# fogleman/sdf

Hardware: AMD Instinct MI355X
Metric: grid voxels/sec (sampled + meshed), canonical CSG example (higher is better)
Workload: dtype f64; 1 GPU; example @ samples=2**27 -> 512x512x512 grid, sparse=True, batch_size=32; batches=4096, skipped=2352, empty=120, nonempty=1624, triangles=2945152, parallelism=single GPU

## Files before the change

sdf_amd/csrc/sdf_device.h:

```cpp
#pragma once
#include <hip/hip_runtime.h>
#include <stdint.h>
#include <type_traits>

#include "sdf_interp.h"
#include "sdf_mc33.h"
#include "sdf_interval.h"
#include "sdf_slab.h"

namespace sdfk {

struct McTables {
    unsigned char ntri[256];
    unsigned char amb[256];
    signed char tri[256][16];
    signed char mc33[MC33_FLAT_SIZE];
};

struct MeshCounters {
    unsigned long long n_pruned;
    unsigned long long n_eval;
    unsigned int work_counter;
    unsigned int overflow;
    unsigned int n_empty, n_nonempty;
    unsigned long long n_ambiguous;
    unsigned long long n_sampled;
    unsigned long long total;
    unsigned long long cell_cursor;
    unsigned long long list_cursor;
    unsigned long long t_first_inv, t_last, clk_cycles, clk_ticks;
    unsigned long long n_raw;
    int nwork, work_begin, work_end, pad_;
};
enum { MESH_COUNTERS_RESET_BYTES = 112 };

struct GridDesc {
    const double *X, *Y, *Z;
    int nx, ny, nz;
    int bs;
    int nbx, nby, nbz;
};

struct MeshArgs {
    GridDesc g;
    const McTables *mc;
    const int *worklist;
    unsigned char *kinds;
    unsigned long long *status;
    double *out;
    unsigned long long out_cap;
    MeshCounters *ctr;
    int bits_off;
    int list_off;
    int list_cap;
    unsigned long long *prof;
    int tape_stride;
    int n_instr;
    float *park;
    int park_cap;
    unsigned park_spins;
    const unsigned char *cull;
    int slot_bytes;
    int stage_off;
    int compact;
    double *xf;
    int xf_cap;
    float *raw;
    long long raw_cap;
    int twopass;
    struct ItemDesc *desc;
    unsigned *cells;
    unsigned *tlist;
    unsigned long long cells_cap, tlist_cap;
    const int *block_item;
    const int *order;
    int tail;
};
enum { MESH_TAIL_MAX = 255 };

struct ItemDesc {
    unsigned ntri, ncells;
    unsigned long long list_off, cell_off;
    double xf[6];
};

enum { MESH_PARK_DEPTH = 16 };
enum { MESH_LDS_SUMS2 = 128, MESH_LDS_NTRI = 192, MESH_LDS_AXES = MESH_LDS_NTRI + 256, MESH_LDS_PEND = MESH_LDS_AXES + 800, MESH_LDS_TRI = MESH_LDS_PEND + 64 * MESH_PARK_DEPTH,
       MESH_LDS_VOL = MESH_LDS_TRI + 256 * 5 * 2 };

__device__ __forceinline__ void batch_origin(const GridDesc &g, int b, int &ox, int &oy, int &oz, int &lx, int &ly, int &lz) {
    const int ibz = b % g.nbz, iby = (b / g.nbz) % g.nby, ibx = b / (g.nbz * g.nby);
    ox = ibx * g.bs; oy = iby * g.bs; oz = ibz * g.bs;
    lx = min(g.bs + 1, g.nx - ox); ly = min(g.bs + 1, g.ny - oy); lz = min(g.bs + 1, g.nz - oz);
}

__device__ __forceinline__ int fast_div(int i, float inv_d) { return (int)(((float)i + 0.5f) * inv_d); }

template <int BLOCK>
__device__ __forceinline__ int block_exclusive_scan(int v, int *wave_sums, int &total) {
    const int lane = threadIdx.x & 63, wid = threadIdx.x >> 6;
    int inc = v;
    inc += __builtin_amdgcn_update_dpp(0, inc, 0x111, 0xf, 0xf, false);
    inc += __builtin_amdgcn_update_dpp(0, inc, 0x112, 0xf, 0xf, false);
    inc += __builtin_amdgcn_update_dpp(0, inc, 0x114, 0xf, 0xf, false);
    inc += __builtin_amdgcn_update_dpp(0, inc, 0x118, 0xf, 0xf, false);
    inc += __builtin_amdgcn_update_dpp(0, inc, 0x142, 0xa, 0xf, false);
    inc += __builtin_amdgcn_update_dpp(0, inc, 0x143, 0xc, 0xf, false);
    if (lane == 63) wave_sums[wid] = inc;
    __syncthreads();
    int base = 0, tot = 0;
#pragma unroll
    for (int w = 0; w < BLOCK / 64; w++) { const int s = wave_sums[w]; if (w < wid) base += s; tot += s; }
    total = tot;
    __syncthreads();
    return base + inc - v;
}

template <int BLOCK>
__device__ __forceinline__ int block_exclusive_scan1(int v, int *wave_sums, int &total) {
    int t = threadIdx.x;
    asm volatile("" : "+v"(t));
    const int lane = t & 63, wid = __builtin_amdgcn_readfirstlane(t >> 6);
    int inc = v;
    inc += __builtin_amdgcn_update_dpp(0, inc, 0x111, 0xf, 0xf, false);
    inc += __builtin_amdgcn_update_dpp(0, inc, 0x112, 0xf, 0xf, false);
    inc += __builtin_amdgcn_update_dpp(0, inc, 0x114, 0xf, 0xf, false);
    inc += __builtin_amdgcn_update_dpp(0, inc, 0x118, 0xf, 0xf, false);
    inc += __builtin_amdgcn_update_dpp(0, inc, 0x142, 0xa, 0xf, false);
    inc += __builtin_amdgcn_update_dpp(0, inc, 0x143, 0xc, 0xf, false);
    if (lane == 63) wave_sums[wid] = inc;
    __syncthreads();
    static_assert(BLOCK / 64 <= 16, "a row of 16 lanes holds the wave totals");
    const int l16 = lane & 15;
    int tot = l16 < BLOCK / 64 ? wave_sums[l16] : 0, base = l16 < wid ? tot : 0;
    tot += __builtin_amdgcn_update_dpp(0, tot, 0x111, 0xf, 0xf, false);   base += __builtin_amdgcn_update_dpp(0, base, 0x111, 0xf, 0xf, false);
    tot += __builtin_amdgcn_update_dpp(0, tot, 0x112, 0xf, 0xf, false);   base += __builtin_amdgcn_update_dpp(0, base, 0x112, 0xf, 0xf, false);
    tot += __builtin_amdgcn_update_dpp(0, tot, 0x114, 0xf, 0xf, false);   base += __builtin_amdgcn_update_dpp(0, base, 0x114, 0xf, 0xf, false);
    tot += __builtin_amdgcn_update_dpp(0, tot, 0x118, 0xf, 0xf, false);   base += __builtin_amdgcn_update_dpp(0, base, 0x118, 0xf, 0xf, false);
    total = __builtin_amdgcn_readlane(tot, 15);
    return __builtin_amdgcn_readlane(base, 15) + inc - v;
}

template <int BLOCK>
__device__ __forceinline__ int block_exclusive_count(bool p, int *wave_sums, int &total) {
    const unsigned long long m = __ballot(p);
    const int below = (int)__builtin_amdgcn_mbcnt_hi((unsigned)(m >> 32), __builtin_amdgcn_mbcnt_lo((unsigned)m, 0u));
    const int wid = threadIdx.x >> 6;
    if ((threadIdx.x & 63) == 0) wave_sums[wid] = __popcll(m);
    __syncthreads();
    int base = 0, tot = 0;
#pragma unroll
    for (int w = 0; w < BLOCK / 64; w++) { const int s = wave_sums[w]; if (w < wid) base += s; tot += s; }
    total = tot;
    __syncthreads();
    return base + below;
}

__device__ __forceinline__ unsigned plane_bits(const float *v, int s0, int s1) {
    return (v[0] > 0.0f ? 1u : 0u) | (v[s1] > 0.0f ? 2u : 0u) | (v[s0] > 0.0f ? 4u : 0u) | (v[s0 + s1] > 0.0f ? 8u : 0u);
}
__device__ __forceinline__ unsigned spread4(unsigned s) { return (s & 1u) | ((s & 2u) << 1) | ((s & 4u) << 2) | ((s & 8u) << 3); }

__device__ __forceinline__ unsigned cell_config(const unsigned long long *rb, int i2) {
    unsigned cfg = 0;
#pragma unroll
    for (int q = 0; q < 4; q++) cfg |= ((unsigned)(rb[q] >> i2) & 3u) << (2 * q);
    return cfg;
}

#ifndef SDF_TAPE_WARM
#define SDF_TAPE_WARM 1
#endif
#ifndef SDF_FAST_VERTEX
#define SDF_FAST_VERTEX 1
#endif
__device__ __forceinline__ float mc_edge_pos(double vlo, double vhi, double ibase) {
    const double eps = 2.220446049250313e-16;
    const double a = eps + fabs(vlo), b = eps + fabs(vhi);
    float pf;
#if SDF_FAST_VERTEX
    const double sab = a + b;
    double r = __builtin_amdgcn_rcp(sab);
    r = fma(fma(-sab, r, 1.0), r, r);
    r = fma(fma(-sab, r, 1.0), r, r);
    double tq = a * r;
    tq = fma(fma(-sab, tq, a), r, tq);
    const double q = ibase + tq;
    const float f_lo = (float)(q - 0x1p-44), f_hi = (float)(q + 0x1p-44);
    pf = f_lo;
    if (__builtin_expect(!(f_lo == f_hi), 0))
#endif
    {
        const double wlo = 1.0 / a, whi = 1.0 / b;
        const double t = whi / (wlo + whi);
        pf = (float)(ibase + t);
    }
    return pf;
}
__device__ __forceinline__ void mc_vertex(const float *v, int s0, int s1, int i0, int i1, int i2, int e, float *o) {
    const int axis = e >> 2, oa = (e >> 1) & 1, ob = e & 1;
    int o0, o1, o2, stride;
    if (axis == 0) { o0 = 0; o1 = oa; o2 = ob; stride = s0; }
    else if (axis == 1) { o0 = oa; o1 = 0; o2 = ob; stride = s1; }
    else { o0 = oa; o1 = ob; o2 = 0; stride = 1; }
    const int base = o0 * s0 + o1 * s1 + o2;
    const float pf = mc_edge_pos((double)v[base], (double)v[base + stride], (double)(axis == 0 ? i0 : (axis == 1 ? i1 : i2)));
    o[0] = axis == 0 ? pf : (float)(i0 + o0); o[1] = axis == 1 ? pf : (float)(i1 + o1); o[2] = axis == 2 ? pf : (float)(i2 + o2);
}

struct TileView {
    const float *smp;
    const unsigned *colinfo;
    int lyz, lz;
    bool sparse;
    __device__ __forceinline__ float at(int ix, int iy, int iz) const {
        if (!sparse) return smp[ix * lyz + iy * lz + iz];
        const unsigned c = colinfo[(ix >> 1) * 17 + (iy >> 1)];
        const int k = (int)(c >> 17) + __popc(c & ((1u << (iz >> 1)) - 1u));
        return smp[8 * k + ((ix & 1) << 2) + ((iy & 1) << 1) + (iz & 1)];
    }
    __device__ __forceinline__ void cell(int i0, int i1, int i2, float *c8) const {
#pragma unroll
        for (int q = 0; q < 8; q++) c8[q] = at(i0 + (q >> 2), i1 + ((q >> 1) & 1), i2 + (q & 1));
    }
};
__device__ __forceinline__ void mc_vertex_view(const TileView &vw, int i0, int i1, int i2, int e, float *o) {
    const int axis = e >> 2, oa = (e >> 1) & 1, ob = e & 1;
    const int o0 = axis == 0 ? 0 : oa, o1 = axis == 0 ? oa : (axis == 1 ? 0 : ob), o2 = axis == 2 ? 0 : ob;
    const int x = i0 + o0, y = i1 + o1, z = i2 + o2;
    const float vlo = vw.at(x, y, z), vhi = vw.at(x + (axis == 0 ? 1 : 0), y + (axis == 1 ? 1 : 0), z + (axis == 2 ? 1 : 0));
    const float pf = mc_edge_pos((double)vlo, (double)vhi, (double)(axis == 0 ? i0 : (axis == 1 ? i1 : i2)));
    o[0] = axis == 0 ? pf : (float)x; o[1] = axis == 1 ? pf : (float)y; o[2] = axis == 2 ? pf : (float)z;
}

struct Tri16Sink {
    double *out;
    float *raw;
    long long raw_cap;
// ... 56 lines not shown
    bool use_first = true;
    for (unsigned spins = 0; spins < max_spins;) {
        constexpr int NW = 4;
        unsigned long long sw[NW];
        const int nwin = use_first ? 1 : NW;
        if (use_first) sw[0] = first;
        else {
#pragma unroll
            for (int k = 0; k < NW; k++) {
                const int j = idx - 64 * k - lane;
                sw[k] = j >= w_begin ? __hip_atomic_load(&status[j], __ATOMIC_RELAXED, __HIP_MEMORY_SCOPE_AGENT)
                                     : MESH_FLAG_PFX;
            }
        }
        use_first = false;
        bool wait = false;
#pragma unroll
        for (int k = 0; k < NW; k++) {
            if (k >= nwin || wait) break;
            const unsigned flag = (unsigned)(sw[k] >> 62);
            const unsigned long long pending = __ballot(flag == 0), is_pfx = __ballot(flag == 2);
            if (is_pfx) {
                const int p = __ffsll((long long)is_pfx) - 1;
                if (pending & ((1ull << p) - 1ull)) { wait = true; break; }
                acc += lane <= p ? (sw[k] & MESH_VAL_MASK) : 0ull;
                const unsigned long long excl = wave_sum_u64(acc);
                if (lane == 0) __hip_atomic_store(&status[w], MESH_FLAG_PFX | (excl + total), __ATOMIC_RELAXED, __HIP_MEMORY_SCOPE_AGENT);
                return excl;
            }
            if (pending) { wait = true; break; }
            acc += sw[k] & MESH_VAL_MASK;
            idx -= 64;
        }
        if (wait) { __builtin_amdgcn_s_sleep(1); spins++; }
    }
    return max_spins < (1u << 24) ? MESH_NOT_READY : ~0ull;
}
#define MESH_SPIN_FOREVER (1u << 24)

__device__ __noinline__ void mc33_triangle(const float *corner, int s0, int s1, int i0, int i1, int i2,
                                           const signed char *tab, int j, float *o) {
    double lv[8];
    int off;
    mc33_load_cell(corner, s0, s1, lv);
    const int n = mc33_cell(lv, tab, &off);
    if (j >= n) { for (int q = 0; q < 9; q++) o[q] = 0.0f; return; }
    const signed char lew_edge[12] = {8, 5, 9, 4, 10, 7, 11, 6, 0, 1, 3, 2};
    for (int q = 0; q < 3; q++) {
        const int e = tab[off + 3 * j + 2 - q];
        if (e == 12) mc33_centre_vertex(lv, i0, i1, i2, o + 3 * q);
        else mc_vertex(corner, s0, s1, i0, i1, i2, lew_edge[e], o + 3 * q);
    }
}

struct TileTasks {
    int lx, ly, lz, lyz, nvox;
    float inv_lyz, inv_lz;
    bool regular;
    int ntask;
    __device__ __forceinline__ TileTasks(int lx_, int ly_, int lz_) : lx(lx_), ly(ly_), lz(lz_) {
        lyz = ly * lz; nvox = lx * lyz;
        inv_lyz = 1.0f / (float)lyz; inv_lz = 1.0f / (float)lz;
        regular = lx == 33 && ly == 33 && lz == 33;
        ntask = regular ? 563 : (nvox + 63) >> 6;
    }
    __device__ __forceinline__ bool sample(int task, int lane, int &ix, int &iy, int &iz) const {
        if (!regular) {
            const int i = min(task * 64 + lane, nvox - 1);
            ix = fast_div(i, inv_lyz); const int r = i - ix * lyz; iy = fast_div(r, inv_lz); iz = r - iy * lz;
            return task * 64 + lane < nvox;
        }
        if (task < 512) { ix = 4 * (task >> 6) + (lane >> 4); iy = 4 * ((task >> 3) & 7) + ((lane >> 2) & 3); iz = 4 * (task & 7) + (lane & 3); return true; }
        if (task < 530) { const int p = min((task - 512) * 64 + lane, 1088); ix = 32; iy = fast_div(p, 1.0f / 33.0f); iz = p - 33 * iy; return (task - 512) * 64 + lane < 1089; }
        if (task < 547) { const int p = min((task - 530) * 64 + lane, 1055); iy = 32; ix = fast_div(p, 1.0f / 33.0f); iz = p - 33 * ix; return (task - 530) * 64 + lane < 1056; }
        const int p = (task - 547) * 64 + lane; iz = 32; ix = p >> 5; iy = p & 31; return true;
    }
};

enum { CULL_UNIT_CAP = 3072, CULL_ULIST = 8, CULL_SBYTES = CULL_ULIST, CULL_SSTATE = CULL_ULIST + 2 * CULL_UNIT_CAP, CULL_COLINFO = CULL_SSTATE + 1024,
       CULL_RECORD = CULL_COLINFO + 1160,
       CULL_MSTATE = CULL_RECORD, CULL_GSTATE = CULL_MSTATE + 64, CULL_ELIST = CULL_GSTATE + 512, CULL_PACC = CULL_ELIST + 1024,
       CULL_SCRATCH = CULL_PACC + 64 };
static_assert(CULL_RECORD % 8 == 0 && CULL_SSTATE % 8 == 0 && CULL_COLINFO % 8 == 0, "the record is copied in words; its state rows are read as u64");
__device__ __forceinline__ bool cull_sample(const unsigned short *units, int task, int lane, int lx, int ly, int lz, int &ix, int &iy, int &iz) {
    const unsigned u = units[8 * task + (lane >> 3)];
    const int x = (int)((u >> 9) & 62u) + ((lane >> 2) & 1), y = (int)((u >> 4) & 62u) + ((lane >> 1) & 1), z = (int)((u << 1) & 62u) + (lane & 1);
    const bool ok = x < lx && y < ly && z < lz;
    ix = ok ? x : 0; iy = ok ? y : 0; iz = ok ? z : 0;
    return ok;
}
template <int BLOCK, bool FULL, bool RARE>
__device__ __forceinline__ int cull_tasks(const uint32_t *wcode, const double *consts, int n_instr_w, int lx, int ly, int lz,
                                       const double *axes, double *ia_state, int ia_bytes, unsigned char *scratch, int *wave_sums,
                                       int ia_np, int ia_nd, unsigned long long *prof = nullptr, int levels = 3) {
    const int tid = threadIdx.x;
    long long tprev = prof ? clock64() : 0;
    unsigned *pacc = reinterpret_cast<unsigned *>(scratch + CULL_PACC);
    if (prof && tid == 0) for (int k = 0; k < 12; k++) pacc[k] = 0;
#define SDF_CULL_PROF(K) do { if (prof && tid == 0) { const long long tn = clock64(); pacc[(K) - 16] += (unsigned)(tn - tprev); tprev = tn; } } while (0)
    const int c0 = lx - 1, c1 = ly - 1, c2 = lz - 1;
    const int per_pass = min(BLOCK, ia_bytes / ((6 * ia_np + 2 * ia_nd) * 8)) & ~63;
    if (c0 <= 0 || c1 <= 0 || c2 <= 0 || per_pass < 64) return -1;
    unsigned short *ulist = reinterpret_cast<unsigned short *>(scratch + CULL_ULIST);
    unsigned char *sstate = scratch + CULL_SBYTES;
    static_assert(2 * CULL_UNIT_CAP >= 4096, "the byte states lie over the unit list");
    unsigned char *mstate = scratch + CULL_MSTATE;
    unsigned char *gstate = scratch + CULL_GSTATE;
    unsigned short *elist = reinterpret_cast<unsigned short *>(scratch + CULL_ELIST);
    auto box_state = [&](int x0, int x1, int y0, int y1, int z0, int z1) -> unsigned char {
        Ival bx{axes[x0], axes[min(x1, c0)]}, by{axes[33 + y0], axes[33 + min(y1, c1)]}, bz{axes[66 + z0], axes[66 + min(z1, c2)]};
        if (bx.lo > bx.hi) { const double t = bx.lo; bx.lo = bx.hi; bx.hi = t; }
        if (by.lo > by.hi) { const double t = by.lo; by.lo = by.hi; by.hi = t; }
        if (bz.lo > bz.hi) { const double t = bz.lo; bz.lo = bz.hi; bz.hi = t; }
        if (ia::bad(bx) || ia::bad(by) || ia::bad(bz)) { bx = by = bz = ia::top(); }
        const Ival v = ia_run_tape<false, FULL, RARE>(wcode, consts, nullptr, nullptr, n_instr_w, bx, by, bz, true,
                                          IaShared{ia_state, ia_np, per_pass}, ia_nd, nullptr);
        return v.lo > 1e-30 ? 1 : (v.hi < -1e-30 ? 2 : 0);
    };
    int phase = 0, e0 = 0, nev = 0;
    for (;;) {
        if (phase == 1 && e0 >= nev) {
            __syncthreads();
            SDF_CULL_PROF(19);
            int nund = 0;
            for (int g0 = 0; levels >= 3 && g0 < 512; g0 += BLOCK) {
                const int gi = g0 + tid;
                const bool und = gi < 512 && gstate[gi] == 0;
                int n;
                const int pos = nund + block_exclusive_count<BLOCK>(und, wave_sums, n);
                if (und) elist[pos] = (unsigned short)gi;
                nund += n;
            }
            for (int h = tid; h < 4096; h += BLOCK) {
                const int h0 = h >> 8, h1 = (h >> 4) & 15, h2 = h & 15;
                const bool exists = 2 * h0 < c0 && 2 * h1 < c1 && 2 * h2 < c2;
                sstate[h] = exists ? gstate[((h0 >> 1) * 8 + (h1 >> 1)) * 8 + (h2 >> 1)] : 1;
            }
            __syncthreads();
            phase = 2; e0 = 0; nev = 8 * nund;
        }
        if (phase == 2 && e0 >= nev) break;
        const bool run = phase == 0 ? tid < 64 : (tid < per_pass && e0 + (tid & ~63) < nev);
        int target = 0, x0, y0, z0, ext;
        bool live;
        if (phase == 0) {
            const int m0 = tid >> 4, m1 = (tid >> 2) & 3, m2 = tid & 3;
            live = 8 * m0 < c0 && 8 * m1 < c1 && 8 * m2 < c2;
            x0 = live ? 8 * m0 : 0; y0 = live ? 8 * m1 : 0; z0 = live ? 8 * m2 : 0; ext = 8;
        } else if (phase == 1) {
            live = e0 + tid < nev;
            target = run ? (int)elist[min(e0 + tid, nev - 1)] : 0;
            x0 = 4 * (target >> 6); y0 = 4 * ((target >> 3) & 7); z0 = 4 * (target & 7); ext = 4;
        } else {
            const int e = min(e0 + tid, nev - 1);
            const int gq = run ? (int)elist[e >> 3] : 0, ch = e & 7;
            const int h0 = 2 * (gq >> 6) + (ch >> 2), h1 = 2 * ((gq >> 3) & 7) + ((ch >> 1) & 1), h2 = 2 * (gq & 7) + (ch & 1);
            live = e0 + tid < nev && 2 * h0 < c0 && 2 * h1 < c1 && 2 * h2 < c2;
            target = (h0 * 16 + h1) * 16 + h2;
            x0 = live ? 2 * h0 : 0; y0 = live ? 2 * h1 : 0; z0 = live ? 2 * h2 : 0; ext = 2;
        }
        if (run) {
            const unsigned char st = box_state(x0, x0 + ext, y0, y0 + ext, z0, z0 + ext);
            if (phase == 0) mstate[tid & 63] = live ? st : 1;
            else if (live) (phase == 1 ? gstate : sstate)[target] = st;
        }
        if (phase != 0) { if (prof && tid == 0) pacc[7]++; e0 += per_pass; continue; }
        SDF_CULL_PROF(17);
        __syncthreads();
        for (int g0 = 0; g0 < 512; g0 += BLOCK) {
            const int gi = g0 + tid;
            const int a0 = gi >> 6, a1 = (gi >> 3) & 7, a2 = gi & 7;
            const bool exists = gi < 512 && 4 * a0 < c0 && 4 * a1 < c1 && 4 * a2 < c2;
            const unsigned char ms = exists ? mstate[((a0 >> 1) * 4 + (a1 >> 1)) * 4 + (a2 >> 1)] : 1;
            if (gi < 512) gstate[gi] = ms;
            int n;
            const int pos = nev + block_exclusive_count<BLOCK>(ms == 0, wave_sums, n);
            if (ms == 0) elist[pos] = (unsigned short)gi;
            nev += n;
        }
        __syncthreads();
        SDF_CULL_PROF(18);
        if (prof && tid == 0) pacc[6] = (unsigned)nev;
        phase = 1; e0 = 0;
    }
    __syncthreads();
    SDF_CULL_PROF(20);
    unsigned short *ub = reinterpret_cast<unsigned short *>(scratch + CULL_GSTATE);
    for (int r = tid; r < 256; r += BLOCK) {
        const unsigned long long lo8 = *reinterpret_cast<const unsigned long long *>(sstate + 16 * r);
        const unsigned long long hi8 = *reinterpret_cast<const unsigned long long *>(sstate + 16 * r + 8);
        unsigned m = 0, pk = 0;
        SDF_UNROLL for (int k = 0; k < 8; k++) { m |= ((lo8 >> (8 * k)) & 255ull) == 0ull ? 1u << k : 0u; pk |= (unsigned)((lo8 >> (8 * k)) & 3ull) << (2 * k); }
        SDF_UNROLL for (int k = 0; k < 8; k++) { m |= ((hi8 >> (8 * k)) & 255ull) == 0ull ? 256u << k : 0u; pk |= (unsigned)((hi8 >> (8 * k)) & 3ull) << (2 * k + 16); }
        ub[r] = (unsigned short)m;
        reinterpret_cast<unsigned *>(scratch + CULL_SSTATE)[r] = pk;
    }
    __syncthreads();
    const int nu0 = (lx + 1) >> 1, nu1 = (ly + 1) >> 1, nu2 = (lz + 1) >> 1;
    int nlisted = 0;
    unsigned *colinfo = reinterpret_cast<unsigned *>(scratch + CULL_COLINFO);
    for (int q0 = 0; q0 < 17 * 17; q0 += BLOCK) {
        const int q = q0 + tid, u0 = q / 17, u1 = q - 17 * u0;
        unsigned um = 0;
        if (q < 17 * 17 && u0 < nu0 && u1 < nu1) {
            unsigned m = 0;
            for (int d0 = 0; d0 < 2; d0++)
                for (int d1 = 0; d1 < 2; d1++) {
                    const int h0 = u0 - d0, h1 = u1 - d1;
                    if (h0 >= 0 && h0 < 16 && h1 >= 0 && h1 < 16) m |= ub[h0 * 16 + h1];
                }
            um = (m | (m << 1)) & ((1u << nu2) - 1u);
        }
        int n;
        int pos = nlisted + block_exclusive_scan<BLOCK>(__popc(um), wave_sums, n);
        nlisted += n;
        if (q < 17 * 17) colinfo[q] = um | ((unsigned)min(pos, 32767) << 17);
        if (nlisted <= CULL_UNIT_CAP) {
            while (um) {
                const int u2 = __ffs((int)um) - 1;
                um &= um - 1u;
                ulist[pos++] = (unsigned short)((u0 << 10) | (u1 << 5) | u2);
            }
        }
    }
    SDF_CULL_PROF(24);
    if (nlisted > CULL_UNIT_CAP) { __syncthreads(); return -1; }
    if (tid < 8 && nlisted + tid < ((nlisted + 7) & ~7)) ulist[nlisted + tid] = 0xFFFFu;
    if (tid == 0) reinterpret_cast<unsigned short *>(scratch)[0] = (unsigned short)nlisted;
    __syncthreads();
    SDF_CULL_PROF(25);
#undef SDF_CULL_PROF
    return (nlisted + 7) >> 3;
}

#ifndef SDF_SOUP_NT
#define SDF_SOUP_NT 0
#endif
#if SDF_SOUP_NT
#define SDF_SOUP_STORE(PTR, VAL) __builtin_nontemporal_store((VAL), (PTR))
#else
#define SDF_SOUP_STORE(PTR, VAL) (*(PTR) = (VAL))
#endif

enum { MESH_SLOT_HDR = 1232, MESH_SLOT_COLINFO = 64, MESH_STAGE_BYTES = 32 * 9 * 4 };

template <typename T, bool FULL, int NP, int ND, int NS, int BLOCK, bool TWOPASS, bool PROF>
__device__ __forceinline__ void mesh_rounds(const uint32_t *__restrict__ code, const T *__restrict__ consts) {
    typedef __attribute__((address_space(4))) const MeshArgs KArgs;
    static_assert(sizeof(const uint32_t *) + sizeof(const T *) == 16 && alignof(MeshArgs) <= 16, "MeshArgs sits at byte 16 of the kernel arguments");
    KArgs *ap = (KArgs *)((__attribute__((address_space(4))) const char *)__builtin_amdgcn_kernarg_segment_ptr() + 16);
#define KA (*ap)
#define SDF_SINK (Tri16Sink{KA.out, KA.raw, KA.raw_cap, &KA.ctr->n_raw})
    typedef Vec<T, NS> V;
    constexpr int RPT = 1024 / BLOCK;
    constexpr int MESH_CELL_CHUNKS = 2;
    extern __shared__ __attribute__((aligned(16))) unsigned char smem[];
    int *wave_sums = reinterpret_cast<int *>(smem);
    int *bcast = wave_sums + 16;
    unsigned char *ntri_lds = smem + MESH_LDS_NTRI;
    double *axes = reinterpret_cast<double *>(smem + MESH_LDS_AXES);
    float *vol = reinterpret_cast<float *>(smem + MESH_LDS_VOL);
    unsigned long long *bits = reinterpret_cast<unsigned long long *>(smem + KA.bits_off);
    unsigned *wlist = reinterpret_cast<unsigned *>(smem + KA.list_off);
    int tid = threadIdx.x;
#define SDF_FRESH() do { asm volatile("" : "+v"(tid), "+s"(ap)); \
                         bits = reinterpret_cast<unsigned long long *>(smem + KA.bits_off); wlist = reinterpret_cast<unsigned *>(smem + KA.list_off); } while (0)
#define SDF_PROF_ON (PROF && KA.prof)
    auto grid = [&]() { GridDesc g_; g_.X = KA.g.X; g_.Y = KA.g.Y; g_.Z = KA.g.Z; g_.nx = KA.g.nx; g_.ny = KA.g.ny; g_.nz = KA.g.nz; g_.bs = KA.g.bs;
                        g_.nbx = KA.g.nbx; g_.nby = KA.g.nby; g_.nbz = KA.g.nbz; return g_; };
    unsigned short *tri_lds = reinterpret_cast<unsigned short *>(smem + MESH_LDS_TRI);

    if (tid < 256) ntri_lds[tid] = (unsigned char)(KA.mc->ntri[tid] | (KA.mc->amb[tid] << 7));
    if (!TWOPASS)
        for (int i = tid; i < 256 * 5; i += BLOCK) {
            const int cfg = i / 5, j = i - 5 * cfg;
            const signed char *t3 = &KA.mc->tri[cfg][3 * j];
            tri_lds[i] = (unsigned short)(((unsigned)t3[0] & 15u) | (((unsigned)t3[1] & 15u) << 4) | (((unsigned)t3[2] & 15u) << 8));
        }

    for (int i = tid; i < (int)((KA.list_off - KA.bits_off) >> 3); i += BLOCK) bits[i] = 0ull;
    const int work_begin = KA.ctr->work_begin, work_end = KA.ctr->work_end;
    if (SDF_PROF_ON && tid == 0) KA.prof[64 + 4 * blockIdx.x] = wall_clock64();
    if (tid == 0) {
        const unsigned long long tw = wall_clock64();
        atomicMax(&KA.ctr->t_first_inv, ~tw);
        if (blockIdx.x == 0) { KA.ctr->clk_cycles = (unsigned long long)clock64(); KA.ctr->clk_ticks = tw; }
    }
    long long tprev = SDF_PROF_ON ? clock64() : 0;
#define SDF_PROF(K) do { if (SDF_PROF_ON && tid == 0) { const long long tn = clock64(); atomicAdd(&KA.prof[K], (unsigned long long)(tn - tprev)); tprev = tn; } } while (0)
    auto settle = [&](int w_, unsigned long long excl, unsigned long long total_) {
        if (excl == ~0ull) atomicOr(&KA.ctr->overflow, 2u);
        else if (excl + total_ > KA.out_cap) atomicOr(&KA.ctr->overflow, 1u);
        if (w_ == work_end - 1 && excl != ~0ull) KA.ctr->total = excl + total_;
    };
    auto my_park = [&]() -> float * { return KA.park ? KA.park + (size_t)blockIdx.x * (size_t)MESH_PARK_DEPTH * (size_t)KA.park_cap * 9 : nullptr; };
    int pq_head = 0, pq_count = 0;
    unsigned char *pend_base = smem + MESH_LDS_PEND;
    auto pend_xf = [&](int k) { return reinterpret_cast<double *>(pend_base + 64 * k); };
    auto pend_wt = [&](int k) { return reinterpret_cast<int *>(pend_base + 64 * k + 48); };
    auto place_parked = [&](unsigned long long pre_pend, bool must, int need) {
        bool first = true;
        while (pq_count > 0) {
            const int pend_w = uni(pend_wt(pq_head)[0]), pend_total = uni(pend_wt(pq_head)[1]);
            const bool block = must || pq_count > MESH_PARK_DEPTH - need;
            if (tid < 64) {
                const unsigned long long pre = first ? pre_pend : lookback_prefetch(KA.status, pend_w, work_begin);
                const unsigned long long excl = ordered_base(KA.status, pend_w, work_begin, (unsigned long long)pend_total,
// ... 674 lines not shown
```

sdf_amd/csrc/sdf_prepass.hip:

```cpp
#include <hip/hip_runtime.h>

#include <algorithm>

#include "sdf_prune.h"
#include "sdf_plain.h"
#include "sdf_internal.h"

using namespace sdfk;

enum { SKIP_BATCHES_PER_BLOCK = 7 * (256 / 64) };
template <typename T, bool FULL, bool RARE>
__device__ __forceinline__ void skip_body(const uint32_t *__restrict__ code, const T *__restrict__ consts, GridDesc g,
                                              int nbatches, unsigned char *__restrict__ kinds, const PruneArgs &pa,
                                              const double *__restrict__ c64, const uint16_t *__restrict__ rstart,
                                              const uint16_t *__restrict__ lstart, double *prune_lds, int skip_b0) {
    if ((int)blockIdx.x >= pa.first_block) {
        prune_block<FULL, RARE>(code, c64, rstart, lstart, pa, g, nbatches, (int)blockIdx.x - pa.first_block, prune_lds);
        return;
    }
    const int lane = threadIdx.x & 63, slot = min(lane / 9, 6), l = lane - 9 * slot;
    const int b = skip_b0 + ((int)blockIdx.x * (256 / 64) + (int)(threadIdx.x >> 6)) * 7 + slot;
    const bool live = b < nbatches && l < 9;
    int ox = 0, oy = 0, oz = 0, lx = 1, ly = 1, lz = 1;
    if (b < nbatches) batch_origin(g, b, ox, oy, oz, lx, ly, lz);
    double x0 = 0, x1 = 0, y0 = 0, y1 = 0, z0 = 0, z1 = 0;
    if (b < nbatches) {
        x0 = g.X[ox]; x1 = g.X[ox + lx - 1]; y0 = g.Y[oy]; y1 = g.Y[oy + ly - 1]; z0 = g.Z[oz]; z1 = g.Z[oz + lz - 1];
    }
    const double cx = (x0 + x1) / 2, cy = (y0 + y1) / 2, cz = (z0 + z1) / 2;
    double px = cx, py = cy, pz = cz;
    if (l >= 1) { const int k = l - 1; px = (k & 4) ? x1 : x0; py = (k & 2) ? y1 : y0; pz = (k & 1) ? z1 : z0; }
    T v = T(0);
    if (live) v = run_tape1<T, FULL>(code, consts, (T)px, (T)py, (T)pz);
    const int base = 9 * slot;
    const T vc = __shfl(v, base, 64);
    const T v1 = __shfl(v, base + 1, 64);
    const bool pos = v1 > T(0);
    const bool ok = pos ? (v > T(0)) : (v < T(0));
    const unsigned long long m = __ballot(ok);
    const bool all_same = ((m >> (base + 1)) & 0xFFull) == 0xFFull;
    if (b < nbatches && l == 0) {
        const double r = fabs((double)vc);
        const double d = sqrt(((cx - x0) * (cx - x0) + (cy - y0) * (cy - y0)) + (cz - z0) * (cz - z0));
        const bool skip = !(r <= d) && all_same;
        kinds[b] = skip ? 0 : 255;
    }
}

template <typename T, bool FULL>
__global__ __launch_bounds__(256) void k_skip(const uint32_t *__restrict__ code, const T *__restrict__ consts, GridDesc g,
                                              int nbatches, unsigned char *__restrict__ kinds, PruneArgs pa,
                                              const double *__restrict__ c64, const uint16_t *__restrict__ rstart, const uint16_t *__restrict__ lstart,
                                              int skip_b0) {
    extern __shared__ double prune_lds[];
    skip_body<T, FULL, false>(code, consts, g, nbatches, kinds, pa, c64, rstart, lstart, prune_lds, skip_b0);
}
template <typename T, bool FULL>
__global__ __launch_bounds__(256) void k_skip_rare(const uint32_t *__restrict__ code, const T *__restrict__ consts, GridDesc g,
                                                   int nbatches, unsigned char *__restrict__ kinds, PruneArgs pa,
                                                   const double *__restrict__ c64, const uint16_t *__restrict__ rstart, const uint16_t *__restrict__ lstart,
                                                   int skip_b0) {
    extern __shared__ double prune_lds[];
    skip_body<T, FULL, true>(code, consts, g, nbatches, kinds, pa, c64, rstart, lstart, prune_lds, skip_b0);
}

template <bool FULL, bool RARE>
__global__ __launch_bounds__(PRUNE_BLOCK) void k_prune_list(const uint32_t *__restrict__ code, GridDesc g, int nbatches, PruneArgs pa,
                                                               const double *__restrict__ c64, const uint16_t *__restrict__ rstart,
                                                               const uint16_t *__restrict__ lstart) {
    extern __shared__ double prune_list_lds[];
    if ((long long)blockIdx.x * (PRUNE_BLOCK / 8) >= (long long)(pa.ctr->work_end - pa.ctr->work_begin)) return;
    prune_block<FULL, RARE>(code, c64, rstart, lstart, pa, g, nbatches, (int)blockIdx.x, prune_list_lds);
}

#define CULL_BLOCK 256
template <bool FULL, bool RARE, int CB = CULL_BLOCK>
__device__ __forceinline__ void cull_body(const uint32_t *__restrict__ code, const double *__restrict__ consts, GridDesc g,
                                                     const int *__restrict__ worklist, const MeshCounters *__restrict__ ctr,
                                                     int tape_stride, int n_instr, int ia_np, int ia_nd, int ia_bytes,
                                                     unsigned char *__restrict__ out, unsigned char *cull_smem, unsigned long long *prof,
                                                     int *__restrict__ order, int tail_max, int levels) {
    int *wave_sums = reinterpret_cast<int *>(cull_smem);
    double *axes = reinterpret_cast<double *>(cull_smem + 64);
    unsigned char *scratch = cull_smem + 896;
    double *ia_state = reinterpret_cast<double *>(cull_smem + 896 + CULL_SCRATCH);
    const int tid = threadIdx.x;
    const long long tstart = prof ? clock64() : 0;
    asm volatile("" :: "s"(g.X), "s"(g.Y), "s"(g.Z), "s"(g.nx), "s"(g.ny), "s"(g.nz), "s"(g.nby), "s"(g.nbz), "s"(g.bs));
    const int w = ctr->work_begin + (int)blockIdx.x;
    if (w >= ctr->work_end) return;
    long long t_ctr = 0, t_b = 0;
    if (prof) asm volatile("s_memtime %0\n\ts_waitcnt lgkmcnt(0)" : "=s"(t_ctr) : "s"(w) : "memory");
    const int b = __builtin_amdgcn_readfirstlane(worklist[w]);
    if (prof) asm volatile("s_memtime %0\n\ts_waitcnt lgkmcnt(0)" : "=s"(t_b) : "s"(b) : "memory");
    int ox, oy, oz, lx, ly, lz;
    batch_origin(g, b, ox, oy, oz, lx, ly, lz);
    long long t_org = 0;
    if (prof) asm volatile("s_memtime %0\n\ts_waitcnt lgkmcnt(0)" : "=s"(t_org) : "s"(ox), "s"(oy), "s"(oz), "s"(lx) : "memory");
    for (int i = tid; i < 99; i += CB) {
        const int ax = i < 33 ? 0 : (i < 66 ? 1 : 2), k = i - 33 * ax;
        const double *src = ax == 0 ? g.X + ox : (ax == 1 ? g.Y + oy : g.Z + oz);
        if (k < (ax == 0 ? lx : (ax == 1 ? ly : lz))) axes[i] = src[k];
    }
    long long t_ax = 0, t_bar = 0;
    if (prof) asm volatile("s_waitcnt vmcnt(0) lgkmcnt(0)\n\ts_memtime %0\n\ts_waitcnt lgkmcnt(0)" : "=s"(t_ax) : "s"(b) : "memory");
    __syncthreads();
    if (prof) asm volatile("s_memtime %0\n\ts_waitcnt lgkmcnt(0)" : "=s"(t_bar) : "s"(b) : "memory");
    const uint32_t *wcode = code + (size_t)b * (size_t)tape_stride * 2;
    const int n_instr_w = tape_stride ? (int)reinterpret_cast<const unsigned long long *>(wcode)[tape_stride - 1] : n_instr;
    long long tstart1 = 0;
    if (prof) asm volatile("s_waitcnt vmcnt(0) lgkmcnt(0)\n\ts_memtime %0\n\ts_waitcnt lgkmcnt(0)" : "=s"(tstart1) : "s"(n_instr_w) : "memory");
    const int ntl = cull_tasks<CB, FULL, RARE>(wcode, consts, n_instr_w, lx, ly, lz, axes, ia_state, ia_bytes, scratch, wave_sums, ia_np, ia_nd, prof, levels);
    const long long tw = prof ? clock64() : 0;
    if (tid == 0 && ntl < 0) reinterpret_cast<unsigned short *>(scratch)[0] = (unsigned short)0xFFFF;
    __syncthreads();
    {
        unsigned *rec = reinterpret_cast<unsigned *>(out + (size_t)w * CULL_RECORD);
        const unsigned *src = reinterpret_cast<const unsigned *>(scratch);
        const int nwords = ntl < 0 ? 1 : (CULL_ULIST + 16 * ntl + 3) >> 2;
        for (int i = tid; i < nwords; i += CB) rec[i] = src[i];
        if (ntl >= 0) for (int i = tid; i < (CULL_RECORD - CULL_SSTATE) / 4; i += CB) rec[CULL_SSTATE / 4 + i] = src[CULL_SSTATE / 4 + i];
    }
    if (order && tid == 0) {
        const int tail = min(tail_max, ctr->work_end - ctr->work_begin), tpos = w - (ctr->work_end - tail);
        if (tpos >= 0) order[tpos] = (ntl < 0 ? 563 : ntl) * max(n_instr_w, 1);
    }
    if (prof && tid == 0) {
        const unsigned *pacc = reinterpret_cast<const unsigned *>(scratch + CULL_PACC);
        atomicAdd(&prof[32 + (ntl < 0 ? 9 : min(ntl >> 6, 8))], 1ull);
        atomicAdd(&prof[16], (unsigned long long)(tstart1 - tstart));
        atomicAdd(&prof[26], (unsigned long long)(t_ctr - tstart));
        atomicAdd(&prof[27], (unsigned long long)(t_b - t_ctr));
        atomicAdd(&prof[28], (unsigned long long)(t_ax - t_org));
        atomicAdd(&prof[30], (unsigned long long)(t_org - t_b));
        atomicAdd(&prof[29], (unsigned long long)(t_bar - t_ax));
        atomicAdd(&prof[21], (unsigned long long)(clock64() - tw));
        for (int k = 1; k < 10; k++) if (k != 5) atomicAdd(&prof[16 + k], (unsigned long long)pacc[k]);
    }
}

template <bool FULL, bool RARE, int CB = CULL_BLOCK>
__global__ __launch_bounds__(CB) void k_cull(const uint32_t *__restrict__ code, const double *__restrict__ consts, GridDesc g,
                                                     const int *__restrict__ worklist, const MeshCounters *__restrict__ ctr,
                                                     int tape_stride, int n_instr, int ia_np, int ia_nd, int ia_bytes,
                                                     unsigned char *__restrict__ out, unsigned long long *prof,
                                                     int *__restrict__ order, int tail_max, int levels) {
    extern __shared__ __attribute__((aligned(16))) unsigned char cull_smem[];
    cull_body<FULL, RARE, CB>(code, consts, g, worklist, ctr, tape_stride, n_instr, ia_np, ia_nd, ia_bytes, out, cull_smem, prof, order, tail_max, levels);
}
__global__ __launch_bounds__(CULL_BLOCK) __attribute__((amdgpu_waves_per_eu(6, 8))) void k_cull_lean(const uint32_t *__restrict__ code, const double *__restrict__ consts, GridDesc g,
                                                     const int *__restrict__ worklist, const MeshCounters *__restrict__ ctr,
                                                     int tape_stride, int n_instr, int ia_np, int ia_nd, int ia_bytes,
                                                     unsigned char *__restrict__ out, unsigned long long *prof,
                                                     int *__restrict__ order, int tail_max, int levels) {
    extern __shared__ __attribute__((aligned(16))) unsigned char cull_smem[];
    cull_body<false, false>(code, consts, g, worklist, ctr, tape_stride, n_instr, ia_np, ia_nd, ia_bytes, out, cull_smem, prof, order, tail_max, levels);
}
__global__ __launch_bounds__(128) __attribute__((amdgpu_waves_per_eu(6, 8))) void k_cull_lean128(const uint32_t *__restrict__ code, const double *__restrict__ consts, GridDesc g,
                                                     const int *__restrict__ worklist, const MeshCounters *__restrict__ ctr,
                                                     int tape_stride, int n_instr, int ia_np, int ia_nd, int ia_bytes,
                                                     unsigned char *__restrict__ out, unsigned long long *prof,
                                                     int *__restrict__ order, int tail_max, int levels) {
    extern __shared__ __attribute__((aligned(16))) unsigned char cull_smem[];
    cull_body<false, false, 128>(code, consts, g, worklist, ctr, tape_stride, n_instr, ia_np, ia_nd, ia_bytes, out, cull_smem, prof, order, tail_max, levels);
}


int enqueue_skip(sdf_tape *t, const double *d_axes, int nx, int ny, int nz, int bs, int b0, int b1, int precision,
                 unsigned char *d_kinds, hipStream_t st) {
    if (b1 <= b0) return 0;
    GridDesc g;
    grid_desc(nx, ny, nz, bs, g);
    g.X = d_axes; g.Y = d_axes + nx; g.Z = d_axes + nx + ny;
    PruneArgs pa = {};
    pa.first_block = 0x7fffffff;
    const unsigned blocks = (unsigned)((b1 - b0 + SKIP_BATCHES_PER_BLOCK - 1) / SKIP_BATCHES_PER_BLOCK);
    LAUNCH_TAPE_ON(st, k_skip, dim3(blocks), dim3(256), 0, t, precision, g, b1, d_kinds, pa, (const double *)t->d_c64,
                   (const uint16_t *)t->d_rstart, (const uint16_t *)t->d_lstart, b0);
    HIPCHK(hipGetLastError());
    return 0;
}

int enqueue_prepass(const GenCall &call, sdf_mesh *m, int nb, int tape_stride, hipStream_t st) {
    sdf_tape *t = call.tape;
    sdf_ctx *c = t->ctx;
    const GridDesc &g = m->g;
    const int sparse = call.sparse, precision = call.precision;
    const bool pruning = tape_stride != 0;
    const uint32_t n_instr = t->n_words / 2;
    PruneArgs pa = {};
    pa.first_block = 0x7fffffff;
    const bool prune_listed = pruning && sparse && (nb >= c->prune_list_min || call.shard_count > 1);
    unsigned skip_blocks = (sparse && !call.d_kinds) ? (unsigned)((nb + SKIP_BATCHES_PER_BLOCK - 1) / SKIP_BATCHES_PER_BLOCK) : 0u, prune_blocks = 0;
    size_t prune_lds = 0;
    if (pruning) {
        if (m->prune.ensure((size_t)nb * 64) || m->tapes.ensure((size_t)nb * tape_stride * 8)) return 1;
        pa.n_instr = (int)n_instr; pa.n_p = std::max(t->n_p, 1u); pa.n_d = std::max(t->n_d, 1u);
        pa.masks_out = (uint32_t *)m->prune.p; pa.tapes_out = (unsigned long long *)m->tapes.p; pa.tape_stride = tape_stride;
        pa.zero_off = t->n_consts;
        prune_lds = prune_lds_bytes(pa.n_p, pa.n_d);
        if (!prune_listed) {
            pa.first_block = (int)skip_blocks;
            prune_blocks = (unsigned)(((long long)nb * 8 + PRUNE_BLOCK - 1) / PRUNE_BLOCK);
        }
    }
    if (skip_blocks + prune_blocks) {
        if (prune_lds > 32768 && prune_blocks) {
            const void *fn = t->ia_rare ? (t->full ? reinterpret_cast<const void *>(k_skip_rare<double, true>) : reinterpret_cast<const void *>(k_skip_rare<double, false>))
                                        : (t->full ? reinterpret_cast<const void *>(k_skip<double, true>) : reinterpret_cast<const void *>(k_skip<double, false>));
// ... 54 lines not shown
```

Measured before the change: 664.1 billion voxels/s.

## Pair-pack block scans, vectorize cull state expansion, and widen record copy

Replaces the ballot-based block count with the DPP scan, packing two 16-bit counts per word so each scan covers two groups. The double-buffered wave-sum slots remove the trailing barrier. The group-to-subgroup state expansion and the undecided/state gathers now use 64-bit bit-twiddling instead of per-byte loops. The record write-out uses 16-byte rows directly from LDS without an extra barrier, and the tape-length load is hoisted before the first barrier to hide its latency. The packed counts and alternating sum buffers assume bounded counts and block sizes, which adds some fragility.

```diff
diff --git a/sdf_amd/csrc/sdf_device.h b/sdf_amd/csrc/sdf_device.h
--- a/sdf_amd/csrc/sdf_device.h
+++ b/sdf_amd/csrc/sdf_device.h
@@ -97,26 +97,6 @@
 __device__ __forceinline__ int fast_div(int i, float inv_d) { return (int)(((float)i + 0.5f) * inv_d); }
 
 template <int BLOCK>
-__device__ __forceinline__ int block_exclusive_scan(int v, int *wave_sums, int &total) {
-    const int lane = threadIdx.x & 63, wid = threadIdx.x >> 6;
-    int inc = v;
-    inc += __builtin_amdgcn_update_dpp(0, inc, 0x111, 0xf, 0xf, false);
-    inc += __builtin_amdgcn_update_dpp(0, inc, 0x112, 0xf, 0xf, false);
-    inc += __builtin_amdgcn_update_dpp(0, inc, 0x114, 0xf, 0xf, false);
-    inc += __builtin_amdgcn_update_dpp(0, inc, 0x118, 0xf, 0xf, false);
-    inc += __builtin_amdgcn_update_dpp(0, inc, 0x142, 0xa, 0xf, false);
-    inc += __builtin_amdgcn_update_dpp(0, inc, 0x143, 0xc, 0xf, false);
-    if (lane == 63) wave_sums[wid] = inc;
-    __syncthreads();
-    int base = 0, tot = 0;
-#pragma unroll
-    for (int w = 0; w < BLOCK / 64; w++) { const int s = wave_sums[w]; if (w < wid) base += s; tot += s; }
-    total = tot;
-    __syncthreads();
-    return base + inc - v;
-}
-
-template <int BLOCK>
 __device__ __forceinline__ int block_exclusive_scan1(int v, int *wave_sums, int &total) {
     int t = threadIdx.x;
     asm volatile("" : "+v"(t));
@@ -142,18 +122,10 @@
 }
 
 template <int BLOCK>
-__device__ __forceinline__ int block_exclusive_count(bool p, int *wave_sums, int &total) {
-    const unsigned long long m = __ballot(p);
-    const int below = (int)__builtin_amdgcn_mbcnt_hi((unsigned)(m >> 32), __builtin_amdgcn_mbcnt_lo((unsigned)m, 0u));
-    const int wid = threadIdx.x >> 6;
-    if ((threadIdx.x & 63) == 0) wave_sums[wid] = __popcll(m);
-    __syncthreads();
-    int base = 0, tot = 0;
-#pragma unroll
-    for (int w = 0; w < BLOCK / 64; w++) { const int s = wave_sums[w]; if (w < wid) base += s; tot += s; }
-    total = tot;
-    __syncthreads();
-    return base + below;
+__device__ __forceinline__ int block_exclusive_scan(int v, int *wave_sums, int &total) {
+    const int pos = block_exclusive_scan1<BLOCK>(v, wave_sums, total);
+    if (BLOCK / 64 > 8) __syncthreads();
+    return pos;
 }
 
 __device__ __forceinline__ unsigned plane_bits(const float *v, int s0, int s1) {
@@ -376,6 +348,32 @@
        CULL_MSTATE = CULL_RECORD, CULL_GSTATE = CULL_MSTATE + 64, CULL_ELIST = CULL_GSTATE + 512, CULL_PACC = CULL_ELIST + 1024,
        CULL_SCRATCH = CULL_PACC + 64 };
 static_assert(CULL_RECORD % 8 == 0 && CULL_SSTATE % 8 == 0 && CULL_COLINFO % 8 == 0, "the record is copied in words; its state rows are read as u64");
+static_assert(CULL_SBYTES % 8 == 0 && CULL_GSTATE % 8 == 0, "a row of byte states (eight groups, twice eight sub-groups) is read and written as u64");
+static_assert(CULL_RECORD % 16 == 0 && (CULL_SSTATE + 8) % 16 == 0, "the record goes out in 16-byte rows: the list from its start, states and column words from CULL_SSTATE + 8");
+SDF_IA unsigned long long cull_double_bytes(unsigned long long g) {
+    unsigned long long t = g & 0xFFFFFFFFull;
+    t = (t | (t << 16)) & 0x0000FFFF0000FFFFull;
+    t = (t | (t << 8)) & 0x00FF00FF00FF00FFull;
+    return t | (t << 8);
+}
+SDF_IA unsigned cull_gather_states(unsigned long long w) {
+    unsigned long long t = w & 0x0303030303030303ull;
+    t = (t | (t >> 6)) & 0x000F000F000F000Full;
+    t = (t | (t >> 12)) & 0x000000FF000000FFull;
+    return (unsigned)((t | (t >> 24)) & 0xFFFFull);
+}
+SDF_IA unsigned cull_gather_undecided(unsigned long long w) {
+    unsigned long long t = ~(w | (w >> 1)) & 0x0101010101010101ull;
+    t = (t | (t >> 7)) & 0x0003000300030003ull;
+    t = (t | (t >> 14)) & 0x0000000F0000000Full;
+    return (unsigned)((t | (t >> 28)) & 0xFFull);
+}
+__device__ __forceinline__ int cull_opaque(int t) {
+#if defined(__HIP_DEVICE_COMPILE__)
+    asm volatile("" : "+v"(t));
+#endif
+    return t;
+}
 __device__ __forceinline__ bool cull_sample(const unsigned short *units, int task, int lane, int lx, int ly, int lz, int &ix, int &iy, int &iz) {
     const unsigned u = units[8 * task + (lane >> 3)];
     const int x = (int)((u >> 9) & 62u) + ((lane >> 2) & 1), y = (int)((u >> 4) & 62u) + ((lane >> 1) & 1), z = (int)((u << 1) & 62u) + (lane & 1);
@@ -411,24 +409,41 @@
                                           IaShared{ia_state, ia_np, per_pass}, ia_nd, nullptr);
         return v.lo > 1e-30 ? 1 : (v.hi < -1e-30 ? 2 : 0);
     };
+    auto group_of_box = [&](int gi) -> unsigned char {
+        const int a0 = gi >> 6, a1 = (gi >> 3) & 7, a2 = gi & 7;
+        return 4 * a0 < c0 && 4 * a1 < c1 && 4 * a2 < c2 ? mstate[((a0 >> 1) * 4 + (a1 >> 1)) * 4 + (a2 >> 1)] : (unsigned char)1;
+    };
+    static_assert(17 * 17 * 17 < 65536 && 512 % (2 * BLOCK) == 0 && BLOCK <= 512, "two counts to a word, whole pairs of groups, two halves of wave totals");
+#define SDF_CULL_SUMS(I0) (wave_sums + 8 * (((I0) / (2 * BLOCK)) & 1))
     int phase = 0, e0 = 0, nev = 0;
     for (;;) {
         if (phase == 1 && e0 >= nev) {
             __syncthreads();
             SDF_CULL_PROF(19);
+            const int t = cull_opaque(tid);
             int nund = 0;
-            for (int g0 = 0; levels >= 3 && g0 < 512; g0 += BLOCK) {
-                const int gi = g0 + tid;
-                const bool und = gi < 512 && gstate[gi] == 0;
+            for (int g0 = 0; levels >= 3 && g0 < 512; g0 += 2 * BLOCK) {
+                const int ga = g0 + t, gb = ga + BLOCK;
+                const bool und_a = gstate[ga] == 0, und_b = gstate[gb] == 0;
                 int n;
-                const int pos = nund + block_exclusive_count<BLOCK>(und, wave_sums, n);
-                if (und) elist[pos] = (unsigned short)gi;
-                nund += n;
-            }
-            for (int h = tid; h < 4096; h += BLOCK) {
-                const int h0 = h >> 8, h1 = (h >> 4) & 15, h2 = h & 15;
-                const bool exists = 2 * h0 < c0 && 2 * h1 < c1 && 2 * h2 < c2;
-                sstate[h] = exists ? gstate[((h0 >> 1) * 8 + (h1 >> 1)) * 8 + (h2 >> 1)] : 1;
+                const int pre = block_exclusive_scan<BLOCK>((und_a ? 1 : 0) | (und_b ? 1 << 16 : 0), SDF_CULL_SUMS(g0), n);
+                if (und_a) elist[nund + (pre & 0xFFFF)] = (unsigned short)ga;
+                if (und_b) elist[nund + (n & 0xFFFF) + (pre >> 16)] = (unsigned short)gb;
+                nund += (n & 0xFFFF) + (n >> 16);
+            }
+            const int n2 = min((c2 + 1) >> 1, 16);
+            const unsigned long long ones = 0x0101010101010101ull;
+            const unsigned long long keep_lo = n2 >= 8 ? ~0ull : (1ull << (8 * n2)) - 1ull, keep_hi = n2 >= 16 ? ~0ull : (n2 > 8 ? (1ull << (8 * (n2 - 8))) - 1ull : 0ull);
+            for (int r = t; r < 256; r += BLOCK) {
+                const int h0 = r >> 4, h1 = r & 15;
+                unsigned long long lo = ones, hi = ones;
+                if (2 * h0 < c0 && 2 * h1 < c1) {
+                    const unsigned long long g = *reinterpret_cast<const unsigned long long *>(gstate + ((h0 >> 1) * 8 + (h1 >> 1)) * 8);
+                    lo = (cull_double_bytes(g) & keep_lo) | (ones & ~keep_lo);
+                    hi = (cull_double_bytes(g >> 32) & keep_hi) | (ones & ~keep_hi);
+                }
+                *reinterpret_cast<unsigned long long *>(sstate + 16 * r) = lo;
+                *reinterpret_cast<unsigned long long *>(sstate + 16 * r + 8) = hi;
             }
             __syncthreads();
             phase = 2; e0 = 0; nev = 8 * nund;
@@ -461,16 +476,16 @@
         if (phase != 0) { if (prof && tid == 0) pacc[7]++; e0 += per_pass; continue; }
         SDF_CULL_PROF(17);
         __syncthreads();
-        for (int g0 = 0; g0 < 512; g0 += BLOCK) {
-            const int gi = g0 + tid;
-            const int a0 = gi >> 6, a1 = (gi >> 3) & 7, a2 = gi & 7;
-            const bool exists = gi < 512 && 4 * a0 < c0 && 4 * a1 < c1 && 4 * a2 < c2;
-            const unsigned char ms = exists ? mstate[((a0 >> 1) * 4 + (a1 >> 1)) * 4 + (a2 >> 1)] : 1;
-            if (gi < 512) gstate[gi] = ms;
+        const int t = cull_opaque(tid);
+        for (int g0 = 0; g0 < 512; g0 += 2 * BLOCK) {
+            const int ga = g0 + t, gb = ga + BLOCK;
+            const unsigned char ms_a = group_of_box(ga), ms_b = group_of_box(gb);
+            gstate[ga] = ms_a; gstate[gb] = ms_b;
             int n;
-            const int pos = nev + block_exclusive_count<BLOCK>(ms == 0, wave_sums, n);
-            if (ms == 0) elist[pos] = (unsigned short)gi;
-            nev += n;
+            const int pre = block_exclusive_scan<BLOCK>((ms_a == 0 ? 1 : 0) | (ms_b == 0 ? 1 << 16 : 0), SDF_CULL_SUMS(g0), n);
+            if (ms_a == 0) elist[nev + (pre & 0xFFFF)] = (unsigned short)ga;
+            if (ms_b == 0) elist[nev + (n & 0xFFFF) + (pre >> 16)] = (unsigned short)gb;
+            nev += (n & 0xFFFF) + (n >> 16);
         }
         __syncthreads();
         SDF_CULL_PROF(18);
@@ -483,40 +498,44 @@
     for (int r = tid; r < 256; r += BLOCK) {
         const unsigned long long lo8 = *reinterpret_cast<const unsigned long long *>(sstate + 16 * r);
         const unsigned long long hi8 = *reinterpret_cast<const unsigned long long *>(sstate + 16 * r + 8);
-        unsigned m = 0, pk = 0;
-        SDF_UNROLL for (int k = 0; k < 8; k++) { m |= ((lo8 >> (8 * k)) & 255ull) == 0ull ? 1u << k : 0u; pk |= (unsigned)((lo8 >> (8 * k)) & 3ull) << (2 * k); }
-        SDF_UNROLL for (int k = 0; k < 8; k++) { m |= ((hi8 >> (8 * k)) & 255ull) == 0ull ? 256u << k : 0u; pk |= (unsigned)((hi8 >> (8 * k)) & 3ull) << (2 * k + 16); }
-        ub[r] = (unsigned short)m;
-        reinterpret_cast<unsigned *>(scratch + CULL_SSTATE)[r] = pk;
+        ub[r] = (unsigned short)(cull_gather_undecided(lo8) | (cull_gather_undecided(hi8) << 8));
+        reinterpret_cast<unsigned *>(scratch + CULL_SSTATE)[r] = cull_gather_states(lo8) | (cull_gather_states(hi8) << 16);
     }
     __syncthreads();
     const int nu0 = (lx + 1) >> 1, nu1 = (ly + 1) >> 1, nu2 = (lz + 1) >> 1;
     int nlisted = 0;
     unsigned *colinfo = reinterpret_cast<unsigned *>(scratch + CULL_COLINFO);
-    for (int q0 = 0; q0 < 17 * 17; q0 += BLOCK) {
-        const int q = q0 + tid, u0 = q / 17, u1 = q - 17 * u0;
-        unsigned um = 0;
-        if (q < 17 * 17 && u0 < nu0 && u1 < nu1) {
-            unsigned m = 0;
-            for (int d0 = 0; d0 < 2; d0++)
-                for (int d1 = 0; d1 < 2; d1++) {
-                    const int h0 = u0 - d0, h1 = u1 - d1;
-                    if (h0 >= 0 && h0 < 16 && h1 >= 0 && h1 < 16) m |= ub[h0 * 16 + h1];
-                }
-            um = (m | (m << 1)) & ((1u << nu2) - 1u);
-        }
+    auto column_units = [&](int q) -> unsigned {
+        const int u0 = q / 17, u1 = q - 17 * u0;
+        if (q >= 17 * 17 || u0 >= nu0 || u1 >= nu1) return 0u;
+        unsigned m = 0;
+        for (int d0 = 0; d0 < 2; d0++)
+            for (int d1 = 0; d1 < 2; d1++) {
+                const int h0 = u0 - d0, h1 = u1 - d1;
+                if (h0 >= 0 && h0 < 16 && h1 >= 0 && h1 < 16) m |= ub[h0 * 16 + h1];
+            }
+        return (m | (m << 1)) & ((1u << nu2) - 1u);
+    };
+    auto list_column = [&](int q, unsigned um, int pos) {
+        const int u0 = q / 17, u1 = q - 17 * u0;
+        while (um) {
+            const int u2 = __ffs((int)um) - 1;
+            um &= um - 1u;
+            ulist[pos++] = (unsigned short)((u0 << 10) | (u1 << 5) | u2);
+        }
+    };
+    for (int q0 = 0; q0 < 17 * 17; q0 += 2 * BLOCK) {
+        const int qa = q0 + tid, qb = qa + BLOCK;
+        const unsigned um_a = column_units(qa), um_b = column_units(qb);
         int n;
-        int pos = nlisted + block_exclusive_scan<BLOCK>(__popc(um), wave_sums, n);
-        nlisted += n;
-        if (q < 17 * 17) colinfo[q] = um | ((unsigned)min(pos, 32767) << 17);
-        if (nlisted <= CULL_UNIT_CAP) {
-            while (um) {
-                const int u2 = __ffs((int)um) - 1;
-                um &= um - 1u;
-                ulist[pos++] = (unsigned short)((u0 << 10) | (u1 << 5) | u2);
-            }
-        }
-    }
+        const int pre = block_exclusive_scan<BLOCK>(__popc(um_a) | (__popc(um_b) << 16), SDF_CULL_SUMS(q0), n);
+        const int pos_a = nlisted + (pre & 0xFFFF), pos_b = nlisted + (n & 0xFFFF) + (pre >> 16);
+        nlisted += (n & 0xFFFF) + (n >> 16);
+        if (qa < 17 * 17) colinfo[qa] = um_a | ((unsigned)min(pos_a, 32767) << 17);
+        if (qb < 17 * 17) colinfo[qb] = um_b | ((unsigned)min(pos_b, 32767) << 17);
+        if (nlisted <= CULL_UNIT_CAP) { list_column(qa, um_a, pos_a); list_column(qb, um_b, pos_b); }
+    }
+#undef SDF_CULL_SUMS
     SDF_CULL_PROF(24);
     if (nlisted > CULL_UNIT_CAP) { __syncthreads(); return -1; }
     if (tid < 8 && nlisted + tid < ((nlisted + 7) & ~7)) ulist[nlisted + tid] = 0xFFFFu;
diff --git a/sdf_amd/csrc/sdf_prepass.hip b/sdf_amd/csrc/sdf_prepass.hip
--- a/sdf_amd/csrc/sdf_prepass.hip
+++ b/sdf_amd/csrc/sdf_prepass.hip
@@ -87,12 +87,16 @@
     const int tid = threadIdx.x;
     const long long tstart = prof ? clock64() : 0;
     asm volatile("" :: "s"(g.X), "s"(g.Y), "s"(g.Z), "s"(g.nx), "s"(g.ny), "s"(g.nz), "s"(g.nby), "s"(g.nbz), "s"(g.bs));
-    const int w = ctr->work_begin + (int)blockIdx.x;
-    if (w >= ctr->work_end) return;
+    const int work_begin = ctr->work_begin, work_end = ctr->work_end;
+    const int w = work_begin + (int)blockIdx.x;
+    if (w >= work_end) return;
+    const int tpos = w - (work_end - min(tail_max, work_end - work_begin));
     long long t_ctr = 0, t_b = 0;
     if (prof) asm volatile("s_memtime %0\n\ts_waitcnt lgkmcnt(0)" : "=s"(t_ctr) : "s"(w) : "memory");
     const int b = __builtin_amdgcn_readfirstlane(worklist[w]);
     if (prof) asm volatile("s_memtime %0\n\ts_waitcnt lgkmcnt(0)" : "=s"(t_b) : "s"(b) : "memory");
+    const uint32_t *wcode = code + (size_t)b * (size_t)tape_stride * 2;
+    const int n_instr_w = tape_stride ? (int)reinterpret_cast<const unsigned long long *>(wcode)[tape_stride - 1] : n_instr;
     int ox, oy, oz, lx, ly, lz;
     batch_origin(g, b, ox, oy, oz, lx, ly, lz);
     long long t_org = 0;
@@ -104,27 +108,24 @@
     }
     long long t_ax = 0, t_bar = 0;
     if (prof) asm volatile("s_waitcnt vmcnt(0) lgkmcnt(0)\n\ts_memtime %0\n\ts_waitcnt lgkmcnt(0)" : "=s"(t_ax) : "s"(b) : "memory");
+    asm volatile("" :: "s"(n_instr_w));
     __syncthreads();
     if (prof) asm volatile("s_memtime %0\n\ts_waitcnt lgkmcnt(0)" : "=s"(t_bar) : "s"(b) : "memory");
-    const uint32_t *wcode = code + (size_t)b * (size_t)tape_stride * 2;
-    const int n_instr_w = tape_stride ? (int)reinterpret_cast<const unsigned long long *>(wcode)[tape_stride - 1] : n_instr;
     long long tstart1 = 0;
     if (prof) asm volatile("s_waitcnt vmcnt(0) lgkmcnt(0)\n\ts_memtime %0\n\ts_waitcnt lgkmcnt(0)" : "=s"(tstart1) : "s"(n_instr_w) : "memory");
     const int ntl = cull_tasks<CB, FULL, RARE>(wcode, consts, n_instr_w, lx, ly, lz, axes, ia_state, ia_bytes, scratch, wave_sums, ia_np, ia_nd, prof, levels);
     const long long tw = prof ? clock64() : 0;
-    if (tid == 0 && ntl < 0) reinterpret_cast<unsigned short *>(scratch)[0] = (unsigned short)0xFFFF;
-    __syncthreads();
-    {
-        unsigned *rec = reinterpret_cast<unsigned *>(out + (size_t)w * CULL_RECORD);
-        const unsigned *src = reinterpret_cast<const unsigned *>(scratch);
-        const int nwords = ntl < 0 ? 1 : (CULL_ULIST + 16 * ntl + 3) >> 2;
-        for (int i = tid; i < nwords; i += CB) rec[i] = src[i];
-        if (ntl >= 0) for (int i = tid; i < (CULL_RECORD - CULL_SSTATE) / 4; i += CB) rec[CULL_SSTATE / 4 + i] = src[CULL_SSTATE / 4 + i];
-    }
-    if (order && tid == 0) {
-        const int tail = min(tail_max, ctr->work_end - ctr->work_begin), tpos = w - (ctr->work_end - tail);
-        if (tpos >= 0) order[tpos] = (ntl < 0 ? 563 : ntl) * max(n_instr_w, 1);
-    }
+    unsigned char *rec = out + (size_t)w * CULL_RECORD;
+    if (ntl < 0) {
+        if (tid == 0) reinterpret_cast<unsigned short *>(rec)[0] = (unsigned short)0xFFFF;
+    } else {
+        constexpr int REST = CULL_SSTATE + 8, REST_ROWS = (CULL_RECORD - REST) / 16;
+        for (int i = tid; i < ntl; i += CB) reinterpret_cast<uint4 *>(rec)[i] = reinterpret_cast<const uint4 *>(scratch)[i];
+        for (int i = tid; i < REST_ROWS; i += CB) reinterpret_cast<uint4 *>(rec + REST)[i] = reinterpret_cast<const uint4 *>(scratch + REST)[i];
+        if (tid == CB - 1) reinterpret_cast<unsigned long long *>(rec)[2 * ntl] = reinterpret_cast<const unsigned long long *>(scratch)[2 * ntl];
+        if (tid == CB - 2) reinterpret_cast<unsigned long long *>(rec + CULL_SSTATE)[0] = reinterpret_cast<const unsigned long long *>(scratch + CULL_SSTATE)[0];
+    }
+    if (order && tid == 0 && tpos >= 0) order[tpos] = (ntl < 0 ? 563 : ntl) * max(n_instr_w, 1);
     if (prof && tid == 0) {
         const unsigned *pacc = reinterpret_cast<const unsigned *>(scratch + CULL_PACC);
         atomicAdd(&prof[32 + (ntl < 0 ? 9 : min(ntl >> 6, 8))], 1ull);
```

Result: faster. 680.4 billion voxels/s, median of 6 (+2.4%).
